# Shimly-2/DRL-on-robot-arm

Measured on AMD Instinct MI355X. Metric: env-steps/sec at N parallel envs (rl_reach_env), higher is better.
Workload: dtype f64

## Files before the change

__graft_entry__.py:

```python
import os
import subprocess
import sys

ROOT = os.path.dirname(os.path.abspath(__file__))
PKG = os.path.join(ROOT, "drl-on-robot-arm_amd")
for p in (ROOT, PKG):
    if p not in sys.path:
        sys.path.insert(0, p)


def build() -> None:
    subprocess.check_call(["make", "-C", PKG, "-j", str(min(8, os.cpu_count() or 1))], stdout=subprocess.DEVNULL)
    from oracle import oracle as _orc
    _orc.build()
    import armenv
    from armenv import _lib
    lib = _lib.load()
    assert lib.armenv_abi_version() == _lib.ABI_VERSION
    from armenv import envs


def smoke() -> None:
    import numpy as np
    import torch
    from armenv import envs
    from oracle import oracle as O

    n = 256
    env = envs.BatchedReachEnv(n, device="cuda:0", seed=1, auto_reset=False)
    assert env.kernel_name == "reach_step<f64,kuka>", env.kernel_name
    chain, cfg = O.make_chain("kuka"), O.default_config()
    st = O.ReachState(n)
    obs = env.reset().cpu().numpy()
    obs_ref = O.reach_reset(chain, cfg, st, seed=1)
    assert np.array_equal(obs[:, 3:], obs_ref[:, 3:]) and np.abs(obs - obs_ref).max() < 1e-6
# ... 19 lines not shown
```

drl-on-robot-arm_amd/armenv/envs/batched.py:

```python
import contextlib
import ctypes as C

import numpy as np
import torch

from .. import _lib as L
from ..spaces import Box
from ..urdf import Chain, builtin_chain


def _ptr(t):
    return None if t is None else C.c_void_p(t.data_ptr())


class BatchedArmEnv:

    task = L.TASK_REACH
    obs_dim = 6
    aux_dim = 0

    def __init__(self, num_envs, device="cuda:0", seed=0, auto_reset=True, precision=64, robot="kuka",
                 chain: Chain = None, env_id_offset=0, fk_path=L.FK_AUTO, **overrides):
        self._h = None
        lib = L.load()
# ... 327 lines not shown
        n, dev = self.num_envs, self.device
        ret = torch.empty(n, dtype=torch.float64, device=dev)
        ln = torch.empty(n, dtype=torch.int32, device=dev)
        su = torch.empty(n, dtype=torch.uint8, device=dev)
        with self._ordered():
            L.check(self._lib.armenv_episode_stats(self._h, _ptr(ret), _ptr(ln), _ptr(su), self._stream()))
        return ret, ln, su

    def summary(self):
        out = torch.empty(8, dtype=torch.float64, device=self.device)
        with self._ordered():
            L.check(self._lib.armenv_summary(self._h, _ptr(out), self._stream()))
        n = out[5]
        return dict(mean_distance=out[0] / n, max_distance=out[1], mean_last_return=out[2] / n, mean_last_len=out[3] / n,
                    last_success_rate=out[4] / n, raw=out)

    def counters(self):
        out = (C.c_uint64 * 16)()
        L.check(self._lib.armenv_counters(self._h, C.byref(out), self._stream()))
        return dict(episodes=out[0], successes=out[1], env_steps=out[2], nonfinite=out[3], ik_updates=out[4],
                    limit_steps=out[5], low_flange_steps=out[6], cap_steps=out[7], illcond_steps=out[8],
                    wave_trips=out[9], wave_rounds=out[10])


class BatchedReachEnv(BatchedArmEnv):
    task = L.TASK_REACH
    obs_dim = 6

    def __init__(self, num_envs, **kw):
        super().__init__(num_envs, **kw)
        lo = [0.2, -0.3, 0.0] * 2
        hi = [0.7, 0.3, 0.55] * 2
        self.observation_space = Box(low=lo, high=hi)


def diana_cam_reach_kinematics():
    import math
    big = 1.0e9
    return dict(chain=builtin_chain("diana").with_base(rpy=(0.0, 0.0, math.pi)), target_quat=[0.0, 0.0, 0.0, 1.0], dv=0.005,
                goal_lo=[0.3, -0.3, 0.0], goal_hi=[0.8, 0.3, 0.55], box_lo=[-big] * 3, box_hi=[big] * 3)


class BatchedPushEnv(BatchedArmEnv):
    task = L.TASK_PUSH
    obs_dim = 9
    aux_dim = 10
# ... 16 lines not shown
```

drl-on-robot-arm_amd/csrc/armenv_engine.h:

```cpp
#pragma once
#include <hip/hip_runtime.h>

#include <algorithm>
#include <cmath>
#include <cstdarg>
#include <cstdio>
#include <cstring>
#include <memory>
#include <new>
#include <string>
#include <type_traits>

#include "armenv_env.h"

int armenv_fail(int code, const char *fmt, ...) __attribute__((format(printf, 2, 3), visibility("hidden")));
#define fail armenv_fail

#define HIP_TRY(expr)                                                                            \
  do {                                                                                           \
    hipError_t e_ = (expr);                                                                      \
    if (e_ != hipSuccess) return fail(ARMENV_EHIP, "%s failed: %s", #expr, hipGetErrorString(e_)); \
  } while (0)

struct DeviceGuard {
// ... 62 lines not shown
                        double *trig, hipStream_t s) = 0;
  virtual int set_state(const double *q, const float *goal, const int32_t *step, const uint32_t *episode,
                        const double *ep_return, const double *aux, const double *trig, hipStream_t s) = 0;
  virtual int episode_stats(double *last_return, int32_t *last_len, uint8_t *last_success, hipStream_t s) = 0;
  virtual int episode_returns_f32(float *last_return, hipStream_t s) = 0;
  virtual int counters(uint64_t out[16], hipStream_t s) = 0;
  virtual int summary(double *out_dev, hipStream_t s) = 0;
  virtual const char *name() const = 0;
};

static inline unsigned grid_for(int64_t n, int block) { return (unsigned)((n + block - 1) / block); }

static constexpr bool fused_policy(int kind) {
  return kind == ARMENV_POLICY_ACTOR || kind == ARMENV_POLICY_ACTOR_F16X3 || kind == ARMENV_POLICY_DATD3 || kind == ARMENV_POLICY_DADDPG;
}


template <template <class, class, int> class LaneT, class C, typename T> struct Engine final : EngineBase {
  using Lane = LaneT<C, T, 0>;
  using LaneF = LaneT<C, T, 1>;
  using LaneTip = LaneT<C, T, 2>;
  bool fence_on = false;
  bool tip_on = false;
  template <bool kFused = false, class F> void with_build(bool two, F &&f) {
    auto waves = [&](auto *lane) {
      if constexpr (!kFused)
        if (two) return f(lane, std::integral_constant<int, 2>{});
      f(lane, std::integral_constant<int, 1>{});
    };
    if constexpr (kFused) waves((Lane *)nullptr);
    else if (tip_on) waves((LaneTip *)nullptr);
    else if (fence_on) waves((LaneF *)nullptr);
    else waves((Lane *)nullptr);
  }
  EnvParams<T> P{};
  void *pool = nullptr;
  unsigned long long *counter_totals = nullptr;
  double *summary_rows = nullptr;
  static constexpr int block = 256;
  int cus = 256;
  int ready_lanes = 0;
  int straggler_trips = 0;
  int waves_cfg = 0;
  int lanes_cfg = 0;
  bool half_waves() const {
    if (lanes_cfg == 64 || two_waves()) return false;
    if (lanes_cfg == 32) return true;
    return task != ARMENV_TASK_REACH && (P.n + 31) / 32 <= (int64_t)4 * cus;
  }
  static constexpr int task = Lane::kTask;
  std::string kname;

  ~Engine() override {
    if (pool) (void)hipFree(pool);
  }

// ... 70 lines not shown
      P.box_lo[k] = (T)cfg.box_lo[k]; P.box_hi[k] = (T)cfg.box_hi[k];
      K.goal_lo[k] = cfg.goal_lo[k]; K.goal_hi[k] = cfg.goal_hi[k];
    }
    double lim_min = 1e300;
    for (int j = 0; j < NJ; ++j) {
      K.q_init[j] = (T)cfg.q_init[j];
      K.lim[j] = (T)cfg.chain.limit_lo[j];
      K.lim[NJ + j] = (T)cfg.chain.limit_hi[j];
      K.lim[2 * NJ] = (T)cfg.limit_erp;
      const double a = -(double)K.lim[j], b2 = (double)K.lim[NJ + j];
      lim_min = std::fmin(lim_min, std::fmin(a, b2));
    }
    P.ik.lim = cold_dev->lim;
    P.ik.lim_min = (T)(lim_min > 0.0 ? lim_min : -1.0);
    if ((double)P.ik.lim_min > lim_min) P.ik.lim_min = std::nextafter(P.ik.lim_min, (T)0);
    for (int k = 0; k < 4; ++k) P.ik.tq[k] = (T)cfg.target_quat[k];
    P.ik.lambda = (T)cfg.ik_lambda;
    P.ik.residual = (T)cfg.ik_residual;
    P.ik.max_dtheta = (T)cfg.ik_max_dtheta;
    P.ik.max_iters = cfg.ik_max_iters;
    P.ik.exit_mode = cfg.ik_exit_mode;
    P.ik.angle_f32 = cfg.ik_angle_f32;
    P.ik.clamp_limits = cfg.clamp_joint_limits;
    waves_cfg = cfg.rollout_waves_per_simd;
    lanes_cfg = cfg.rollout_lanes_per_wave;
    ready_lanes = cfg.rollout_ready_lanes < 0 ? 0 : (cfg.rollout_ready_lanes > 64 ? 64 : cfg.rollout_ready_lanes);
    straggler_trips = cfg.rollout_straggler_trips < 0 ? 0 : cfg.rollout_straggler_trips;
    tip_on = cfg.ik_tip_offset[0] != 0.0 || cfg.ik_tip_offset[1] != 0.0 || cfg.ik_tip_offset[2] != 0.0 || cfg.fence_counters == 2;
    fence_on = cfg.fence_counters != 0 || tip_on;
    for (int k = 0; k < 3; ++k) P.ik.tip[k] = (T)cfg.ik_tip_offset[k];
    P.ik.fence_pivot = (T)cfg.fence_pivot;
    P.fence_z = (T)cfg.fence_z;
    for (int j = 0; j < NJ; ++j) {
      double R[9];
      rpy_to_mat(cfg.chain.origin_rpy[j], R);
      for (int k = 0; k < 9; ++k) P.chain.R[j][k] = (T)R[k];
      for (int k = 0; k < 3; ++k) P.chain.xyz[j][k] = (T)cfg.chain.origin_xyz[j][k];
    }
    {
      double R[9];
      rpy_to_mat(cfg.chain.base_rpy, R);
      for (int k = 0; k < 9; ++k) P.chain.base_R[k] = (T)R[k];
      for (int k = 0; k < 3; ++k) P.chain.base_p[k] = (T)cfg.chain.base_xyz[k];
    }
    HIP_TRY(hipMemcpy(cold_dev, &K, sizeof K, hipMemcpyHostToDevice));
    hipLaunchKernelGGL((trig_identity_kernel<T>), dim3(grid_for(n, block)), dim3(block), 0, 0, P);
// ... 23 lines not shown
  Launch geometry(Family f) const {
    if (f == Family::RolloutWg) return {dim3(grid_for(P.n, block)), dim3(block), P, false};
    if (two_waves()) return {dim3(grid_for(P.n, block)), dim3(block), P, true};
    const bool h = f != Family::Step && half_waves();
    const int64_t waves = h ? (P.n + 31) / 32 : (P.n + 63) / 64, per_cu = (waves + cus - 1) / cus;
    const int b = 64 * (int)std::min<int64_t>(4, std::max<int64_t>(1, per_cu));
    EnvParams<T> Q = P;
    Q.half_waves = h;
    return {dim3(grid_for(64 * waves, b)), dim3(b), Q, false};
  }
  int step(const StepIO &io, hipStream_t s) override {
    const Launch G = geometry(Family::Step);
    with_build(G.two, [&](auto *lane, auto waves) {
      using LX = std::remove_pointer_t<decltype(lane)>;
      hipLaunchKernelGGL((env_step_kernel<LX, T, decltype(waves)::value>), G.grid, G.block, 0, s, G.P, io);
    });
    HIP_TRY(hipGetLastError());
    return ARMENV_OK;
  }
  template <int POLICY>
  void launch_rollout(Family f, int32_t steps, const float *actions, const StepIO &io0, float *actions_out, hipStream_t s) {
    constexpr bool kFused = fused_policy(POLICY);
    const Launch G = geometry(f);
    with_build<kFused>(G.two, [&](auto *lane, auto waves) {
      using LX = std::remove_pointer_t<decltype(lane)>;
      constexpr int W = decltype(waves)::value;
      if constexpr (!kFused) {
        if (f == Family::RolloutAsync) {
          const int32_t ready = G.P.half_waves ? (ready_lanes + 1) / 2 : ready_lanes;
          hipLaunchKernelGGL((env_rollout_async_kernel<LX, T, POLICY, W>), G.grid, G.block, 0, s, G.P, pol, steps, actions, io0,
                             actions_out, ready, (int32_t)straggler_trips);
          return;
        }
      }
      hipLaunchKernelGGL((env_rollout_kernel<LX, T, POLICY, W>), G.grid, G.block, 0, s, G.P, pol, steps, actions, io0, actions_out);
    });
  }
  int rollout(int32_t steps, const float *actions, const StepIO &io0, float *actions_out, hipStream_t s) override {
    const Family f = ready_lanes > 0 && steps > 1 ? Family::RolloutAsync : Family::Rollout;
    if (actions) launch_rollout<ARMENV_POLICY_EXTERNAL>(f, steps, actions, io0, actions_out, s);
    else if (pol.kind == ARMENV_POLICY_ACTOR) launch_rollout<ARMENV_POLICY_ACTOR>(Family::RolloutWg, steps, actions, io0, actions_out, s);
    else if (pol.kind == ARMENV_POLICY_ACTOR_F16X3) launch_rollout<ARMENV_POLICY_ACTOR_F16X3>(Family::RolloutWg, steps, actions, io0, actions_out, s);
    else if (fused_policy(pol.kind)) launch_rollout<ARMENV_POLICY_DATD3>(Family::RolloutWg, steps, actions, io0, actions_out, s);
    else launch_rollout<ARMENV_POLICY_RANDOM>(f, steps, actions, io0, actions_out, s);
    HIP_TRY(hipGetLastError());
    return ARMENV_OK;
  }
// ... 68 lines not shown
```

drl-on-robot-arm_amd/csrc/armenv_env.h:

```cpp
#pragma once
#include "../../include/armenv.h"
#include "armenv_kin.h"
#include "armenv_actor.h"

using namespace armenv;


template <typename T> struct EnvCold {
  T q_init[NJ];
  T p_init[3];
  T trig_init[2 * NJ];
  T lim[2 * NJ + 1];
  double goal_lo[3], goal_hi[3];
  double push_rest_z, push_place_min, push_place_max, push_place_z;
  uint64_t seed, env_id0;
  int32_t push_model;
  int32_t fall_on;
  int32_t fall_land;
  T fall_c;
  T fall_keep;
  T place_z;
  T tool_radius, tool_below, erp_dt, split, fric_dv, dt;
};

// ... 55 lines not shown
    row[4] += u;
    if (l) row[5] += l;
    if (z) row[6] += z;
    if (c) row[7] += c;
    if (k) row[8] += k;
  }
}
AE_DEV uint32_t wave_max8(uint32_t v) {
  uint32_t m = 0;
  for (int b = 7; b >= 0; --b) { if (__ballot(v >= (m | (1u << b))) != 0ull) m |= 1u << b; }
  return m;
}
AE_DEV void flush_schedule(unsigned long long *counters, uint32_t wave_trips, uint32_t wave_rounds) {
  if (__ffsll((unsigned long long)__ballot(1)) - 1 == (int)(threadIdx.x & 63)) {
    unsigned long long *row = counters + kCounterCols * wave_row();
    row[9] += wave_trips;
    row[10] += wave_rounds;
  }
}
AE_DEV void flush_env_steps(unsigned long long *counters, int64_t i, unsigned long long env_steps) {
  if (i == 0) counters[2] += env_steps;
}

static __global__ __launch_bounds__(256) void counters_sum_kernel(const unsigned long long *rows, int64_t n_rows,
                                                                   unsigned long long *totals) {
  __shared__ unsigned long long part[4][kCounterCols];
  const int col = threadIdx.x & (kCounterCols - 1);
  unsigned long long acc = 0;
  for (int64_t r = threadIdx.x / kCounterCols; r < n_rows; r += 256 / kCounterCols) acc += rows[kCounterCols * r + col];
  for (int o = kCounterCols; o < 64; o <<= 1) acc += __shfl_xor(acc, o);
  if ((threadIdx.x & 63) < kCounterCols) part[threadIdx.x >> 6][col] = acc;
  __syncthreads();
  if (threadIdx.x < kCounterCols) totals[threadIdx.x] = part[0][threadIdx.x] + part[1][threadIdx.x] + part[2][threadIdx.x] + part[3][threadIdx.x];
}

struct ActionPrefetch { float x, y, z; };
AE_DEV void prefetch_issue(const float *src, ActionPrefetch &d) {
  asm volatile("global_load_dword %0, %3, off\n\tglobal_load_dword %1, %3, off offset:4\n\tglobal_load_dword %2, %3, off offset:8"
               : "=a"(d.x), "=a"(d.y), "=a"(d.z) : "v"(src) : "memory");
}
AE_DEV void prefetch_settle(ActionPrefetch &d, float (&out)[3]) {
  asm volatile("s_waitcnt vmcnt(0)\n\tv_accvgpr_read_b32 %0, %3\n\tv_accvgpr_read_b32 %1, %4\n\tv_accvgpr_read_b32 %2, %5"
               : "=v"(out[0]), "=v"(out[1]), "=v"(out[2]) : "a"(d.x), "a"(d.y), "a"(d.z) : "memory");
}

#ifndef ARMENV_TRIG_REDERIVE
// ... 265 lines not shown
        P.last_success[i] = succ ? 1 : 0;
        n_done += 1;
        if (succ) n_succ += 1;
      }
      if (done && P.auto_reset) {
        const uint32_t ep = P.episode[i];
        sample_goal(P, i, ep, g);
        P.episode[i] = ep + 1u;
        static_for<0, 3>([&](auto KI) { constexpr int k = KI; P.goal[(int64_t)k * n + i] = g[k]; });
        const EnvCold<T> &K = *P.cold;
        static_for<0, NJ>([&](auto JI) { constexpr int j = JI; q[j] = K.q_init[j]; });
        static_for<0, NJ>([&](auto JI) { constexpr int j = JI; cq[j] = K.trig_init[j]; sq[j] = K.trig_init[NJ + j]; });
        step = 0;
        ep_ret = T(0);
        store_obs6<T>(io.obs, i, K.p_init, g);
        cur_obs[0] = (float)K.p_init[0]; cur_obs[1] = (float)K.p_init[1]; cur_obs[2] = (float)K.p_init[2];
        if constexpr (CARRY) make_frame(P);
      } else if (rederive) {
        derive_trig();
        if constexpr (CARRY) make_frame(P);
      }
    }
  }
  template <bool CARRY = false, int PEEL = 0>
  AE_DEV int env_step(const EnvParams<T> &P, int64_t i, const T (&a)[3], const StepIO &io, ActionPrefetch *prefetched = nullptr,
                    float (*next_action)[3] = nullptr) {
    T tgt[3];
    step_begin<CARRY>(P, a, tgt);
    const int updates = ik_lockstep<C, T, kMode, PEEL>(P.chain, P.ik, q, tgt, S, cq, sq, minpiv);
    const bool lim_hit = ik_limits<C, T, kMode>(P.chain, P.ik, q, S, cq, sq);
    if (prefetched) prefetch_settle(*prefetched, *next_action);
    step_tail<CARRY>(P, i, io, updates, lim_hit);
    return updates;
  }

  float cur_obs[3];
  AE_DEV void refresh_obs(const EnvParams<T> &P) {
    FKState<T> F;
    fk<C, T>(P.chain, cq, sq, F);
    cur_obs[0] = (float)F.p[0]; cur_obs[1] = (float)F.p[1]; cur_obs[2] = (float)F.p[2];
  }
  AE_DEV void policy_obs(float (&s)[6]) const {
    s[0] = cur_obs[0]; s[1] = cur_obs[1]; s[2] = cur_obs[2]; s[3] = g[0]; s[4] = g[1]; s[5] = g[2];
  }
};

template <bool PICK, typename T>
AE_DEV void cube_sample(const EnvParams<T> &P, int64_t i, uint32_t episode, T (&cube)[3], T (&target)[3]) {
  const EnvCold<T> &K = *P.cold;
  double cx = 0, cy = 0, tx = 0, ty = 0, tz = K.push_place_z;
  constexpr uint32_t kBlocks = PICK ? 4u : 3u;
  for (uint32_t t = 0; t < 1000u; ++t) {
// ... 298 lines not shown
        if (succ) n_succ += 1;
      }
      if (done && P.auto_reset) {
        const uint32_t ep = P.episode[i];
        cube_sample<PICK, T>(P, i, ep, cube, target);
        P.episode[i] = ep + 1u;
        d_last = dist_ct();
        if constexpr (PICK) { grip = T(0); off[0] = off[1] = off[2] = T(0); }
        else { vel[0] = vel[1] = T(0); }
        const EnvCold<T> &K = *P.cold;
        static_for<0, NJ>([&](auto JI) { constexpr int j = JI; q[j] = K.q_init[j]; });
        static_for<0, NJ>([&](auto JI) { constexpr int j = JI; cq[j] = K.trig_init[j]; sq[j] = K.trig_init[NJ + j]; });
        step = 0;
        ep_ret = T(0);
        store_obs9<T>(io.obs, i, K.p_init, cube, target);
        cur_obs[0] = (float)K.p_init[0]; cur_obs[1] = (float)K.p_init[1]; cur_obs[2] = (float)K.p_init[2];
        if constexpr (kCarry) make_frame(P);
      } else if (rederive) {
        derive_trig();
        if constexpr (kCarry) make_frame(P);
      }
    }
  }
  template <bool CARRY = false, int PEEL = 0>
  AE_DEV int env_step(const EnvParams<T> &P, int64_t i, const T (&a)[3], const StepIO &io, ActionPrefetch *prefetched = nullptr,
                    float (*next_action)[3] = nullptr) {
    T tgt[3];
    step_begin<CARRY>(P, a, tgt);
    const int updates = ik_lockstep<C, T, kMode, PEEL>(P.chain, P.ik, q, tgt, S, cq, sq, minpiv);
    const bool lim_hit = ik_limits<C, T, kMode>(P.chain, P.ik, q, S, cq, sq);
    if (prefetched) prefetch_settle(*prefetched, *next_action);
    step_tail<CARRY>(P, i, io, updates, lim_hit);
    return updates;
  }
};
template <class C, typename T, int MODE = 0> using PushLane = CubeLane<C, T, false, MODE>;
template <class C, typename T, int MODE = 0> using PickLane = CubeLane<C, T, true, MODE>;

template <class Lane, typename T>
__global__ __launch_bounds__(256) void env_reset_kernel(EnvParams<T> P, const uint8_t *mask, const float *goal_in, float *obs) {
  const int64_t i = (int64_t)blockIdx.x * blockDim.x + threadIdx.x;
  if (i >= P.n) return;
  if (mask && !mask[i]) return;
  Lane::reset_env(P, i, goal_in, obs);
}

template <class Lane, typename T, int WAVES = 1>
__global__ __launch_bounds__(256) __attribute__((amdgpu_waves_per_eu(WAVES, WAVES))) void env_step_kernel(EnvParams<T> P, StepIO io) {
  TL_STAMP(tl0);
#ifdef ARMENV_TIMELINE
  const unsigned tl_launch = __hip_atomic_load(&g_tl_launch, __ATOMIC_RELAXED, __HIP_MEMORY_SCOPE_AGENT);
#endif
// ... 53 lines not shown
      nw = (int)(((left < (int64_t)blockDim.x ? left : (int64_t)blockDim.x) + 63) >> 6);
      if ((int)(threadIdx.x >> 6) < nw) actor_ring_init(pol.actor_h, w2_ring, nw);
    }
    __syncthreads();
  }
  const int64_t i = kActor ? (int64_t)blockIdx.x * blockDim.x + threadIdx.x : lane_env(P);
  if (i < 0) return;
  if (i >= P.n) return;
  const int64_t n = P.n;
  constexpr int kObs = Lane::kObs;
  Lane L;
  L.load(P, i);
  uint32_t episode = (POLICY != ARMENV_POLICY_EXTERNAL) ? P.episode[i] : 0u;
  if constexpr (kActor) L.refresh_obs(P);
  float an[3] = {0.f, 0.f, 0.f};
  if constexpr (kPrefetch) {
    an[0] = actions[3 * i]; an[1] = actions[3 * i + 1]; an[2] = actions[3 * i + 2];
    asm volatile("" ::"v"(an[0]), "v"(an[1]), "v"(an[2]));
  }
  ActionPrefetch an_next{0.f, 0.f, 0.f};
  [[maybe_unused]] uint32_t w_trips = 0;
  constexpr bool kCarry = !kActor;
  constexpr int kPeel = kActor ? 0 : ARMENV_ROLLOUT_PEEL;
  if constexpr (kCarry) L.make_frame(P);
  for (int32_t t = 0; t < steps; ++t) {
    T a[3];
    if constexpr (kPrefetch) {
      a[0] = (T)an[0]; a[1] = (T)an[1]; a[2] = (T)an[2];
      prefetch_issue(actions + ((int64_t)(t + 1 < steps ? t + 1 : t) * n + i) * 3, an_next);
    } else if constexpr (POLICY == ARMENV_POLICY_EXTERNAL) {
      const float *ap = actions + ((int64_t)t * n + i) * 3;
      a[0] = (T)ap[0]; a[1] = (T)ap[1]; a[2] = (T)ap[2];
    } else {
      float mu[3] = {0.f, 0.f, 0.f};
      if constexpr (POLICY == ARMENV_POLICY_ACTOR) {
        float s[kObs];
        L.policy_obs(s);
        actor_forward_wave<kObs>(pol.actor, w1_lds, s, mu);
      } else if constexpr (POLICY == ARMENV_POLICY_ACTOR_F16X3) {
        float s[kObs];
        L.policy_obs(s);
        actor_forward_wg_f16x3<kObs>(pol.actor, pol.actor_h, w1_lds, w2_ring, nw, s, mu);
      } else if constexpr (kDatd3) {
        float s[kObs], q1, q2;
        int picked;
        L.policy_obs(s);
// ... 6 lines not shown
        float v = fmaf(nz[k], pol.sigma, mu[k]);
        v = fminf(fmaxf(v, -pol.clip), pol.clip);
        a[k] = (T)v;
        an[k] = v;
      });
    }
    StepIO io;
    io.action = nullptr;
    io.obs = io0.obs + (int64_t)t * n * kObs;
    io.reward = io0.reward + (int64_t)t * n;
    io.done = io0.done + (int64_t)t * n;
    io.success = io0.success + (int64_t)t * n;
    io.terminal_obs = io0.terminal_obs ? io0.terminal_obs + (int64_t)t * n * kObs : nullptr;
    if constexpr (Lane::kFence) io.updates = io0.updates ? io0.updates + (int64_t)t * n : nullptr; else io.updates = nullptr;
    if constexpr (kTipOf(Lane::kMode)) io.diag = io0.diag ? io0.diag + (int64_t)t * n * 4 : nullptr; else io.diag = nullptr;
    if (__builtin_expect(actions_out != nullptr, 0)) {
      float *ao = actions_out + ((int64_t)t * n + i) * 3;
      if constexpr (POLICY == ARMENV_POLICY_EXTERNAL) { ao[0] = (float)a[0]; ao[1] = (float)a[1]; ao[2] = (float)a[2]; }
      else { ao[0] = an[0]; ao[1] = an[1]; ao[2] = an[2]; }
    }
    const uint32_t before = L.n_done;
    int upd;
    if constexpr (kPrefetch) {
      upd = L.template env_step<kCarry, kPeel>(P, i, a, io, &an_next, &an);
    } else {
      upd = L.template env_step<kCarry, kPeel>(P, i, a, io);
    }
    if constexpr (Lane::kFence) w_trips += wave_max8((uint32_t)upd + 1u);
    else (void)upd;
    if constexpr (POLICY != ARMENV_POLICY_EXTERNAL) {
      if (L.n_done != before && P.auto_reset) episode += 1u;
    }
  }
  L.store(P, i);
  if constexpr (kRing) actor_ring_drain();
  if constexpr (Lane::kFence) flush_schedule(P.counters, w_trips, (uint32_t)steps);
  flush_env_steps(P.counters, i, (unsigned long long)n * (unsigned long long)steps);
}

template <class Lane, typename T, int POLICY, int WAVES = 1>
__global__ __launch_bounds__(256) __attribute__((amdgpu_waves_per_eu(WAVES, WAVES)))
void env_rollout_async_kernel(EnvParams<T> P, PolicyParams pol, int32_t steps, const float *actions, StepIO io0,
                              float *actions_out, int32_t ready_lanes, int32_t straggler_trips) {
  static_assert(POLICY == ARMENV_POLICY_EXTERNAL || POLICY == ARMENV_POLICY_RANDOM, "no wave-synchronous policy phases here");
  const int64_t i = lane_env(P);
  if (i < 0) return;
  if (i >= P.n) return;
  const int64_t n = P.n;
  constexpr int kObs = Lane::kObs;
  using C = typename Lane::Chain;
  Lane L;
  L.load(P, i);
  uint32_t episode = (POLICY != ARMENV_POLICY_EXTERNAL) ? P.episode[i] : 0u;
  const T res2 = P.ik.residual * P.ik.residual;
  const bool small_steps = P.ik.max_dtheta <= T(0.7854);
  int32_t t = 0;
  bool ready = false;
  T tgt[3], diff2_prev = T(1e60);
  int updates = 0;
  float af[3] = {0.f, 0.f, 0.f};
  auto load_action = [&](int32_t tt) {
    if constexpr (POLICY == ARMENV_POLICY_EXTERNAL) {
      const float *ap = actions + ((int64_t)tt * n + i) * 3;
      af[0] = ap[0]; af[1] = ap[1]; af[2] = ap[2];
    }
  };
  auto begin_step = [&]() {
    T a[3];
    if constexpr (POLICY != ARMENV_POLICY_EXTERNAL) {
      float nz[3];
      policy_noise(P.seed, P.env_id0 + (uint64_t)i, episode - 1u, (uint32_t)L.step, nz);
      static_for<0, 3>([&](auto KI) {
        constexpr int k = KI;
        float v = nz[k] * pol.sigma;
        af[k] = fminf(fmaxf(v, -pol.clip), pol.clip);
      });
    }
    a[0] = (T)af[0]; a[1] = (T)af[1]; a[2] = (T)af[2];
    if (actions_out) {
      float *ao = actions_out + ((int64_t)t * n + i) * 3;
      ao[0] = af[0]; ao[1] = af[1]; ao[2] = af[2];
    }
    L.template step_begin<true>(P, a, tgt);
    diff2_prev = T(1e60);
    updates = 0;
    ready = false;
  };
  load_action(0);
  L.make_frame(P);
  begin_step();
  [[maybe_unused]] uint32_t w_trips = 0, w_rounds = 0;
  for (;;) {
    if constexpr (Lane::kFence) w_trips += __ballot(!ready && t < steps) != 0ull ? 1u : 0u;
    if (!ready && t < steps) ready = ik_trip<C, T, Lane::kMode>(P.chain, P.ik, L.q, tgt, L.S, L.cq, L.sq, diff2_prev, updates, res2, small_steps, L.minpiv);
    const unsigned long long rb = __ballot(ready), ib = __ballot(!ready && t < steps);
    const bool round = straggler_trips > 0 ? __ballot(!ready && t < steps && updates < straggler_trips) == 0ull : __popcll(rb) >= ready_lanes;
    if (round || ib == 0ull) {
      if constexpr (Lane::kFence) w_rounds += rb != 0ull ? 1u : 0u;
      if (ready) {
        if (t + 1 < steps) load_action(t + 1);
        const bool lim_hit = ik_limits<C, T, Lane::kMode>(P.chain, P.ik, L.q, L.S, L.cq, L.sq);
        StepIO io;
        io.action = nullptr;
        io.obs = io0.obs + (int64_t)t * n * kObs;
        io.reward = io0.reward + (int64_t)t * n;
        io.done = io0.done + (int64_t)t * n;
        io.success = io0.success + (int64_t)t * n;
        io.terminal_obs = io0.terminal_obs ? io0.terminal_obs + (int64_t)t * n * kObs : nullptr;
        if constexpr (Lane::kFence) io.updates = io0.updates ? io0.updates + (int64_t)t * n : nullptr; else io.updates = nullptr;
    if constexpr (kTipOf(Lane::kMode)) io.diag = io0.diag ? io0.diag + (int64_t)t * n * 4 : nullptr; else io.diag = nullptr;
        const uint32_t before = L.n_done;
        L.template step_tail<true>(P, i, io, updates, lim_hit);
        if constexpr (POLICY != ARMENV_POLICY_EXTERNAL) {
          if (L.n_done != before && P.auto_reset) episode += 1u;
        }
        ready = false;
        ++t;
        if (t < steps) begin_step();
      }
    }
    if (__ballot(t < steps) == 0ull) break;
  }
  L.store(P, i);
  if constexpr (Lane::kFence) flush_schedule(P.counters, w_trips, w_rounds);
  flush_env_steps(P.counters, i, (unsigned long long)n * (unsigned long long)steps);
}

template <class C, typename T>
__global__ __launch_bounds__(256) void fk_kernel(EnvParams<T> P, int64_t n, const double *q_in, double *pos, double *quat) {
  const int64_t i = (int64_t)blockIdx.x * blockDim.x + threadIdx.x;
  if (i >= n) return;
  T q[NJ];
  static_for<0, NJ>([&](auto JI) { constexpr int j = JI; q[j] = (T)q_in[7 * i + j]; });
  FKState<T> S;
  T cq[NJ], sq[NJ];
  sincos_all<T>(q, cq, sq);
  fk<C, T>(P.chain, cq, sq, S);
  static_for<0, 3>([&](auto KI) { constexpr int k = KI; pos[3 * i + k] = (double)S.p[k]; });
  if (quat) {
    T qc[4];
    quat_from_frame<T>(S.W, qc);
    static_for<0, 4>([&](auto KI) { constexpr int k = KI; quat[4 * i + k] = (double)qc[k]; });
  }
}

template <class C, typename T, int MODE = 0>
__global__ __launch_bounds__(256) void ik_kernel(EnvParams<T> P, int64_t n, const double *q_in, const double *tgt_in,
                                                 double *q_out, int32_t *iters) {
// ... 104 lines not shown
```

drl-on-robot-arm_amd/csrc/armenv_kin.h:

```cpp
#pragma once
#include "armenv_math.h"
#include "chains_builtin.h"

namespace armenv {

constexpr bool kFenceOf(int mode) { return mode >= 1; }
constexpr bool kTipOf(int mode) { return mode == 2; }

template <typename T> struct ChainDev {
  T xyz[NJ][3];
  T R[NJ][9];
  T base_p[3];
  T base_R[9];
};

struct GenericChain {
  static constexpr bool kGeneric = true;
  static constexpr const char *kName = "generic";
};

template <typename T> struct IKParams {
  T tq[4];
  T lambda;
  T residual;
  T max_dtheta;
  int32_t max_iters;
  int32_t exit_mode;
  int32_t angle_f32;
  int32_t clamp_limits;
  int32_t pad0;
// ... 218 lines not shown
template <typename T>
AE_DEV T fast_rcp(T d) {
#ifdef ARMENV_EXACT_RCP
  return T(1) / d;
#endif
  T r = hw_rcp(d);
  r = Mth<T>::fma(Mth<T>::fma(-d, r, T(1)), r, r);
  if constexpr (sizeof(T) == 8) r = Mth<T>::fma(Mth<T>::fma(-d, r, T(1)), r, r);
  return r;
}

template <typename T>
AE_DEV T fast_rsqrt(T x) {
#ifdef ARMENV_EXACT_RSQRT
  return T(1) / Mth<T>::sqrt(x);
#endif
  T r = hw_rsq(x);
  const T hx = T(0.5) * x;
  r = Mth<T>::fma(Mth<T>::fma(-hx * r, r, T(0.5)), r, r);
  if constexpr (sizeof(T) == 8) r = Mth<T>::fma(Mth<T>::fma(-hx * r, r, T(0.5)), r, r);
  return r;
}

template <typename T>
AE_DEV void quat_from_frame(const T (&W)[9], T (&q)[4]) {
  const T m00 = W[0], m10 = W[1], m20 = W[2], m01 = W[3], m11 = W[4], m21 = W[5], m02 = W[6], m12 = W[7], m22 = W[8];
  const T trace = m00 + m11 + m22;
  const bool cw = trace > T(0);
  const bool cz = !cw & (m00 < m11 ? (m11 < m22) : (m00 < m22));
  const bool cy = !cw & !cz & (m00 < m11);
  const T tw = trace + T(1), tz = m22 - m00 - m11 + T(1), ty = m11 - m22 - m00 + T(1), tx = m00 - m11 - m22 + T(1);
  const T t = cw ? tw : (cz ? tz : (cy ? ty : tx));
  const T h = T(0.5) * fast_rsqrt<T>(t);
  const T big = t * h;
  const T d21 = (m21 - m12) * h, d02 = (m02 - m20) * h, d10 = (m10 - m01) * h;
  T s10 = (m10 + m01) * h, s20 = (m20 + m02) * h, s21 = (m21 + m12) * h;
  asm("" : "+v"(s10), "+v"(s20), "+v"(s21));
  q[0] = cw ? d21 : (cz ? s20 : (cy ? s10 : big));
  q[1] = cw ? d02 : (cz ? s21 : (cy ? big : s10));
  q[2] = cw ? d10 : (cz ? big : (cy ? s21 : s20));
  q[3] = cw ? big : (cz ? d10 : (cy ? d02 : d21));
}

AE_DEV double acos_branchfree(double x) {
#ifdef ARMENV_EXACT_ACOS
  return ::acos(x);
#endif
  const double ax = ::fabs(x);
  const bool small = ax < 0.5;
  const double z = small ? x * x : ::fma(-0.5, ax, 0.5);
  double p = ::fma(3.47933107596021167570e-05, z, 7.91534994289814532176e-04);
  p = ::fma(p, z, -4.00555345006794114027e-02);
  p = ::fma(p, z, 2.01212532134862925881e-01);
  p = ::fma(p, z, -3.25565818622400915405e-01);
  p = ::fma(p, z, 1.66666666666666657415e-01);
  p = p * z;
  double q = ::fma(7.70381505559019352791e-02, z, -6.88283971605453293030e-01);
  q = ::fma(q, z, 2.02094576023350569471e+00);
  q = ::fma(q, z, -2.40339491173441421878e+00);
  q = ::fma(q, z, 1.0);
  const double R = p * fast_rcp<double>(q);
  const double sr = z * fast_rsqrt<double>(small ? 1.0 : (z > 0.0 ? z : 1.0));
  const double s = z > 0.0 ? sr : 0.0;
  const double pio2_hi = 1.57079632679489655800e+00, pio2_lo = 6.12323399573676603587e-17;
  const double inner = pio2_hi - (x - ::fma(-x, R, pio2_lo));
  const double w = ::fma(R, s, s);
  const double outer = x < 0.0 ? ::fma(-2.0, w - pio2_lo, 3.14159265358979311600e+00) : 2.0 * w;
  return small ? inner : outer;
}

template <typename T>
AE_DEV void orientation_error(const T (&tq)[4], const T (&qc)[4], int angle_f32, T (&e)[3]) {
  using M = Mth<T>;
  const T bx = -qc[0], by = -qc[1], bz = -qc[2], bw = qc[3];
  const T ax = tq[0], ay = tq[1], az = tq[2], aw = tq[3];
  const T dx = M::fma(aw, bx, M::fma(ax, bw, M::fma(ay, bz, -(az * by))));
  const T dy = M::fma(aw, by, M::fma(ay, bw, M::fma(az, bx, -(ax * bz))));
  const T dz = M::fma(aw, bz, M::fma(az, bw, M::fma(ax, by, -(ay * bx))));
  const T dw = M::fma(aw, bw, -M::fma(ax, bx, M::fma(ay, by, az * bz)));
  if constexpr (sizeof(T) == 4) {
    const T sg = dw < T(0) ? T(-1) : T(1);
    const T n = M::sqrt(M::fma(dx, dx, M::fma(dy, dy, dz * dz)));
    const T ang = T(2) * ::atan2f(n, sg * dw);
    const T k = n > T(1e-30) ? sg * ang / n : T(0);
    e[0] = k * dx; e[1] = k * dy; e[2] = k * dz;
    return;
  }
  const T wc = dw < T(-1) ? T(-1) : (dw > T(1) ? T(1) : dw);
  T angle = T(2) * (T)acos_branchfree((double)wc);
  const T s2 = M::fma(-dw, dw, T(1));
  const T v2 = M::fma(dx, dx, M::fma(dy, dy, dz * dz));
  const bool degenerate = (s2 < T(10) * M::eps) || !(v2 > T(0));
  const T rv = fast_rsqrt<T>(degenerate ? T(1) : v2);
  if (angle_f32) angle = (T)(float)angle;
  angle = angle > M::pi ? angle - T(2) * M::pi : angle;
  if (angle_f32) angle = (T)(float)angle;
  e[0] = degenerate ? angle : angle * (dx * rv);
  e[1] = degenerate ? T(0) : angle * (dy * rv);
  e[2] = degenerate ? T(0) : angle * (dz * rv);
}

template <class C, bool G = C::kGeneric> struct Axis0 { static constexpr int m = 2, sg = 1; };
template <class C> struct Axis0<C, false> { static constexpr int m = C::perm[0][2], sg = C::sgn[0][2]; };
template <class C> constexpr int k0_kind(int row) {
  if (C::kGeneric) return 0;
  const int m = Axis0<C>::m, sg = Axis0<C>::sg;
  if (row < 3) return row == m ? 1 : 0;
  return (row - 3 == m) ? (sg > 0 ? 2 : 3) : 1;
}
template <class C, bool G = C::kGeneric> struct ZKind { static constexpr int of(int, int) { return 0; } };
template <class C> struct ZKind<C, false> { static constexpr int of(int k, int r) { return FkKinds<C>().Ak[k][6 + r]; } };
template <class C> constexpr int col_kind(int k, int row) {
  if (k == 0) return k0_kind<C>(row);
  return row < 3 ? 0 : ZKind<C>::of(k, row - 3);
}
template <class C, typename T, int K, int R, int CC>
AE_DEV T jj_term(T a, T b, T acc) {
  constexpr int ka = col_kind<C>(K, R), kb = col_kind<C>(K, CC);
  if constexpr (ka == 1 || kb == 1) return acc;
  else if constexpr (ka >= 2 && kb >= 2) return acc + ((ka == kb) ? T(1) : T(-1));
  else if constexpr (ka == 2) return acc + b;
  else if constexpr (ka == 3) return acc - b;
  else if constexpr (kb == 2) return acc + a;
  else if constexpr (kb == 3) return acc - a;
  else return Mth<T>::fma(a, b, acc);
}
template <class C, typename T, int MODE = 0>
AE_DEV void dls_update(const FKState<T> &S, const T (&pe)[3], const T (&e)[6], const IKParams<T> &P, T (&dth)[NJ], T &minpiv) {
  using M = Mth<T>;
  constexpr bool FENCE = kFenceOf(MODE);
  constexpr int NL = kTipOf(MODE) ? NJ : NJ - 1;
  T Jl[NL][3];
  static_for<0, NL>([&](auto II) {
    constexpr int i = II;
    const T r0 = pe[0] - S.pj[i][0], r1 = pe[1] - S.pj[i][1], r2 = pe[2] - S.pj[i][2];
    if constexpr (i == 0 && !C::kGeneric) {
      constexpr int m = Axis0<C>::m, sg = Axis0<C>::sg;
      const T r[3] = {r0, r1, r2};
      Jl[0][m] = T(0);
      Jl[0][(m + 1) % 3] = sg > 0 ? -r[(m + 2) % 3] : r[(m + 2) % 3];
      Jl[0][(m + 2) % 3] = sg > 0 ? r[(m + 1) % 3] : -r[(m + 1) % 3];
    } else {
      constexpr int kz0 = ZKind<C>::of(i, 0), kz1 = ZKind<C>::of(i, 1), kz2 = ZKind<C>::of(i, 2);
      constexpr auto neg = [](int k) constexpr { return k < 2 ? k : (k == 2 ? 3 : 2); };
      Jl[i][0] = rot_term<kz1, neg(kz2), T>(r2, S.z[i][1], r1, -S.z[i][2]);
      Jl[i][1] = rot_term<kz2, neg(kz0), T>(r0, S.z[i][2], r2, -S.z[i][0]);
      Jl[i][2] = rot_term<kz0, neg(kz1), T>(r1, S.z[i][0], r0, -S.z[i][1]);
    }
  });
  T A[6][6];
// ... 66 lines not shown
        else if constexpr (kind == 2) { s = first ? y[r] : s + y[r]; first = false; }
        else if constexpr (kind == 3) { s = first ? -y[r] : s - y[r]; first = false; }
      });
    } else if constexpr (i < NL) {
      s = Jl[i][0] * y[0];
      s = M::fma(Jl[i][1], y[1], s);
      s = M::fma(Jl[i][2], y[2], s);
      static_for<0, 3>([&](auto RI) {
        constexpr int r = RI;
        constexpr int kz = ZKind<C>::of(i, r);
        if constexpr (kz == 0) s = M::fma(S.z[i][r], y[3 + r], s);
        else if constexpr (kz == 2) s = s + y[3 + r];
        else if constexpr (kz == 3) s = s - y[3 + r];
      });
    } else {
      s = S.z[i][0] * y[3];
      s = M::fma(S.z[i][1], y[4], s);
      s = M::fma(S.z[i][2], y[5], s);
    }
    dth[i] = s;
    mx = M::fmax(mx, M::fabs(s));
  });
  const bool over = mx > P.max_dtheta;
  const T sc = over ? P.max_dtheta * fast_rcp<T>(over ? mx : T(1)) : T(1);
  static_for<0, NJ>([&](auto II) { constexpr int i = II; dth[i] = dth[i] * sc; });
}

template <typename T, bool START_F32>
AE_DEV void ik_target(const FKState<T> &S, const T (&a)[3], T dv, const T (&box_lo)[3], const T (&box_hi)[3], T (&tgt)[3]) {
  using M = Mth<T>;
  static_for<0, 3>([&](auto KI) {
    constexpr int k = KI;
    T v = M::fma(a[k], dv, START_F32 ? (T)(float)S.p[k] : S.p[k]);
    v = v < box_lo[k] ? box_lo[k] : v;
    v = v > box_hi[k] ? box_hi[k] : v;
    tgt[k] = v;
  });
}
template <class C, typename T, int MODE = 0>
AE_DEV bool ik_stop(const IKParams<T> &P, const T (&tgt)[3], const FKState<T> &S, T diff2_prev, int it, T res2, T (&e)[6], T (&pe)[3],
                    T &diff2) {
  using M = Mth<T>;
  static_for<0, 3>([&](auto RI) {
    constexpr int r = RI;
    if constexpr (kTipOf(MODE)) pe[r] = M::fma(S.W[0 + r], P.tip[0], M::fma(S.W[3 + r], P.tip[1], M::fma(S.W[6 + r], P.tip[2], S.p[r])));
    else pe[r] = S.p[r];
  });
  e[0] = tgt[0] - pe[0];
  e[1] = tgt[1] - pe[1];
  e[2] = tgt[2] - pe[2];
  diff2 = M::fma(e[0], e[0], M::fma(e[1], e[1], e[2] * e[2]));
  int em = P.exit_mode;
  asm("" : "+v"(em));
  const T dtest = em == 0 ? diff2_prev : diff2;
  return (it >= P.max_iters) | !(dtest > res2);
}
template <class C, typename T, int MODE = 0, int SMALL = -1>
AE_DEV void ik_update(const ChainDev<T> &ch, const IKParams<T> &P, T (&q)[NJ], FKState<T> &S, T (&cq)[NJ], T (&sq)[NJ], T (&e)[6],
                      const T (&pe)[3], T diff2, T &diff2_prev, int &it, bool small_steps, T &minpiv) {
  T qc[4], eo[3], dth[NJ];
  quat_from_frame<T>(S.W, qc);
  orientation_error<T>(P.tq, qc, P.angle_f32, eo);
  e[3] = eo[0]; e[4] = eo[1]; e[5] = eo[2];
  dls_update<C, T, MODE>(S, pe, e, P, dth, minpiv);
  static_for<0, NJ>([&](auto II) { constexpr int i = II; q[i] += dth[i]; });
  if constexpr (SMALL >= 0) small_steps = SMALL != 0;
#ifdef ARMENV_EXACT_ROTATE
  small_steps = false;
#endif
  if (__builtin_expect(small_steps, 1)) {
    static_for<0, NJ>([&](auto II) { constexpr int i = II; rotate_small<T>(cq[i], sq[i], dth[i]); });
  } else {
    sincos_all<T>(q, cq, sq);
  }
  diff2_prev = diff2;
  ++it;
  fk<C, T>(ch, cq, sq, S);
}
template <class C, typename T, int MODE = 0, int SMALL = -1>
AE_DEV bool ik_trip(const ChainDev<T> &ch, const IKParams<T> &P, T (&q)[NJ], const T (&tgt)[3], FKState<T> &S, T (&cq)[NJ],
                    T (&sq)[NJ], T &diff2_prev, int &it, T res2, bool small_steps, T &minpiv) {
  T e[6], pe[3], diff2;
  if (ik_stop<C, T, MODE>(P, tgt, S, diff2_prev, it, res2, e, pe, diff2)) return true;
  ik_update<C, T, MODE, SMALL>(ch, P, q, S, cq, sq, e, pe, diff2, diff2_prev, it, small_steps, minpiv);
  return false;
}
template <class C, typename T, int MODE = 0, int PEEL = 0>
AE_DEV int ik_lockstep(const ChainDev<T> &ch, const IKParams<T> &P, T (&q)[NJ], const T (&tgt)[3], FKState<T> &S, T (&cq)[NJ],
                       T (&sq)[NJ], T &minpiv) {
  const T res2 = P.residual * P.residual;
  const bool small_steps = P.max_dtheta <= T(0.7854);
  T diff2_prev = T(1e60);
  int it = 0;
  bool stopped = false;
  static_for<0, PEEL>([&](auto) {
    if (!stopped) stopped = ik_trip<C, T, MODE>(ch, P, q, tgt, S, cq, sq, diff2_prev, it, res2, small_steps, minpiv);
  });
  if (!stopped) while (!ik_trip<C, T, MODE>(ch, P, q, tgt, S, cq, sq, diff2_prev, it, res2, small_steps, minpiv)) {}
  return it;
}

template <class C, typename T, int MODE = 0>
AE_DEV bool ik_limits(const ChainDev<T> &ch, const IKParams<T> &P, T (&q)[NJ], FKState<T> &S, T (&cq)[NJ], T (&sq)[NJ]) {
  using M = Mth<T>;
  constexpr bool FENCE = kFenceOf(MODE);
  bool hit = false;
  if (FENCE || __builtin_expect(P.clamp_limits != 0, 0)) {
    T m = M::fabs(q[0]);
    static_for<1, NJ>([&](auto II) { constexpr int i = II; m = M::fmax(m, M::fabs(q[i])); });
    if (__builtin_expect(m > P.lim_min, 0)) {
      T lo[NJ], hi[NJ];
      static_for<0, NJ>([&](auto II) { constexpr int i = II; lo[i] = P.lim[i]; hi[i] = P.lim[NJ + i]; });
      static_for<0, NJ>([&](auto II) { constexpr int i = II; hit = hit | (q[i] < lo[i]) | (q[i] > hi[i]); });
      if (P.clamp_limits && hit) {
        if (P.clamp_limits == 2) {
          const T erp = P.lim[2 * NJ];
          static_for<0, NJ>([&](auto II) {
            constexpr int i = II;
            q[i] = q[i] < lo[i] ? M::fma(erp, lo[i] - q[i], q[i]) : (q[i] > hi[i] ? M::fma(erp, hi[i] - q[i], q[i]) : q[i]);
          });
        } else {
          static_for<0, NJ>([&](auto II) { constexpr int i = II; q[i] = q[i] < lo[i] ? lo[i] : (q[i] > hi[i] ? hi[i] : q[i]); });
        }
        sincos_all<T>(q, cq, sq);
        fk<C, T>(ch, cq, sq, S);
      }
    }
  }
  return hit;
// ... 28 lines not shown
```

Before: 11.42 billion.

## Add specialized default-IK lane mode with wave-uniform fast paths in IK loop

Adds a lane mode 3 that is selected when the IK configuration matches the defaults (exit mode 0, f32 angle, small max step, no limit clamping). In this mode the exit test, small-step rotation, angle precision and limit check become compile-time constants. It also adds wave-uniform fast paths: the quaternion extraction skips the trace/z branches, acos takes only the large-argument branch, and the dtheta rescale is skipped when no lane in the wave exceeds the cap. The aim is to remove divergent selects and runtime parameter checks from the inner IK loop. The cost is extra template instantiations, a new counter column, and a changed build target.

Result: faster. 11.77 billion, median of 4 (+3.0%).

```diff
diff --git a/__graft_entry__.py b/__graft_entry__.py
--- a/__graft_entry__.py
+++ b/__graft_entry__.py
@@ -10,7 +10,7 @@
 
 
 def build() -> None:
-    subprocess.check_call(["make", "-C", PKG, "-j", str(min(8, os.cpu_count() or 1))], stdout=subprocess.DEVNULL)
+    subprocess.check_call(["make", "-C", PKG, "-j", str(min(8, os.cpu_count() or 1)), "all", "nofast"], stdout=subprocess.DEVNULL)
     from oracle import oracle as _orc
     _orc.build()
     import armenv
diff --git a/drl-on-robot-arm_amd/armenv/envs/batched.py b/drl-on-robot-arm_amd/armenv/envs/batched.py
--- a/drl-on-robot-arm_amd/armenv/envs/batched.py
+++ b/drl-on-robot-arm_amd/armenv/envs/batched.py
@@ -373,6 +373,11 @@
                     limit_steps=out[5], low_flange_steps=out[6], cap_steps=out[7], illcond_steps=out[8],
                     wave_trips=out[9], wave_rounds=out[10])
 
+    def default_ik_env_steps(self):
+        out = (C.c_uint64 * 16)()
+        L.check(self._lib.armenv_counters(self._h, C.byref(out), self._stream()))
+        return int(out[11])
+
 
 class BatchedReachEnv(BatchedArmEnv):
     task = L.TASK_REACH
diff --git a/drl-on-robot-arm_amd/csrc/armenv_engine.h b/drl-on-robot-arm_amd/csrc/armenv_engine.h
--- a/drl-on-robot-arm_amd/csrc/armenv_engine.h
+++ b/drl-on-robot-arm_amd/csrc/armenv_engine.h
@@ -108,7 +108,9 @@
   using LaneTip = LaneT<C, T, 2>;
   bool fence_on = false;
   bool tip_on = false;
-  template <bool kFused = false, class F> void with_build(bool two, F &&f) {
+  using LaneD = LaneT<C, T, 3>;
+  bool default_ik = false;
+  template <bool kFused = false, bool kRollout = false, class F> void with_build(bool two, F &&f) {
     auto waves = [&](auto *lane) {
       if constexpr (!kFused)
         if (two) return f(lane, std::integral_constant<int, 2>{});
@@ -117,7 +119,9 @@
     if constexpr (kFused) waves((Lane *)nullptr);
     else if (tip_on) waves((LaneTip *)nullptr);
     else if (fence_on) waves((LaneF *)nullptr);
-    else waves((Lane *)nullptr);
+    else if (kRollout && default_ik) {
+      if constexpr (kRollout) waves((LaneD *)nullptr);
+    } else waves((Lane *)nullptr);
   }
   EnvParams<T> P{};
   void *pool = nullptr;
@@ -234,6 +238,7 @@
     P.ik.exit_mode = cfg.ik_exit_mode;
     P.ik.angle_f32 = cfg.ik_angle_f32;
     P.ik.clamp_limits = cfg.clamp_joint_limits;
+    default_ik = P.ik.exit_mode == 0 && P.ik.angle_f32 != 0 && P.ik.max_dtheta <= T(0.7854) && P.ik.clamp_limits == 0;
     waves_cfg = cfg.rollout_waves_per_simd;
     lanes_cfg = cfg.rollout_lanes_per_wave;
     ready_lanes = cfg.rollout_ready_lanes < 0 ? 0 : (cfg.rollout_ready_lanes > 64 ? 64 : cfg.rollout_ready_lanes);
@@ -303,7 +308,7 @@
   void launch_rollout(Family f, int32_t steps, const float *actions, const StepIO &io0, float *actions_out, hipStream_t s) {
     constexpr bool kFused = fused_policy(POLICY);
     const Launch G = geometry(f);
-    with_build<kFused>(G.two, [&](auto *lane, auto waves) {
+    with_build<kFused, !kFused>(G.two, [&](auto *lane, auto waves) {
       using LX = std::remove_pointer_t<decltype(lane)>;
       constexpr int W = decltype(waves)::value;
       if constexpr (!kFused) {
diff --git a/drl-on-robot-arm_amd/csrc/armenv_env.h b/drl-on-robot-arm_amd/csrc/armenv_env.h
--- a/drl-on-robot-arm_amd/csrc/armenv_env.h
+++ b/drl-on-robot-arm_amd/csrc/armenv_env.h
@@ -101,6 +101,10 @@
   if (i == 0) counters[2] += env_steps;
 }
 
+AE_DEV void flush_default_ik_steps(unsigned long long *counters, int64_t i, unsigned long long env_steps) {
+  if (i == 0) counters[11] += env_steps;
+}
+
 static __global__ __launch_bounds__(256) void counters_sum_kernel(const unsigned long long *rows, int64_t n_rows,
                                                                    unsigned long long *totals) {
   __shared__ unsigned long long part[4][kCounterCols];
@@ -412,12 +416,12 @@
       }
     }
   }
-  template <bool CARRY = false, int PEEL = 0>
+  template <bool CARRY = false, int PEEL = 0, bool FAST = false>
   AE_DEV int env_step(const EnvParams<T> &P, int64_t i, const T (&a)[3], const StepIO &io, ActionPrefetch *prefetched = nullptr,
                     float (*next_action)[3] = nullptr) {
     T tgt[3];
     step_begin<CARRY>(P, a, tgt);
-    const int updates = ik_lockstep<C, T, kMode, PEEL>(P.chain, P.ik, q, tgt, S, cq, sq, minpiv);
+    const int updates = ik_lockstep<C, T, kMode, PEEL, FAST>(P.chain, P.ik, q, tgt, S, cq, sq, minpiv);
     const bool lim_hit = ik_limits<C, T, kMode>(P.chain, P.ik, q, S, cq, sq);
     if (prefetched) prefetch_settle(*prefetched, *next_action);
     step_tail<CARRY>(P, i, io, updates, lim_hit);
@@ -762,12 +766,12 @@
       }
     }
   }
-  template <bool CARRY = false, int PEEL = 0>
+  template <bool CARRY = false, int PEEL = 0, bool FAST = false>
   AE_DEV int env_step(const EnvParams<T> &P, int64_t i, const T (&a)[3], const StepIO &io, ActionPrefetch *prefetched = nullptr,
                     float (*next_action)[3] = nullptr) {
     T tgt[3];
     step_begin<CARRY>(P, a, tgt);
-    const int updates = ik_lockstep<C, T, kMode, PEEL>(P.chain, P.ik, q, tgt, S, cq, sq, minpiv);
+    const int updates = ik_lockstep<C, T, kMode, PEEL, FAST>(P.chain, P.ik, q, tgt, S, cq, sq, minpiv);
     const bool lim_hit = ik_limits<C, T, kMode>(P.chain, P.ik, q, S, cq, sq);
     if (prefetched) prefetch_settle(*prefetched, *next_action);
     step_tail<CARRY>(P, i, io, updates, lim_hit);
@@ -867,6 +871,7 @@
   [[maybe_unused]] uint32_t w_trips = 0;
   constexpr bool kCarry = !kActor;
   constexpr int kPeel = kActor ? 0 : ARMENV_ROLLOUT_PEEL;
+  constexpr bool kFast = !kActor && !Lane::kFence;
   if constexpr (kCarry) L.make_frame(P);
   for (int32_t t = 0; t < steps; ++t) {
     T a[3];
@@ -919,9 +924,9 @@
     const uint32_t before = L.n_done;
     int upd;
     if constexpr (kPrefetch) {
-      upd = L.template env_step<kCarry, kPeel>(P, i, a, io, &an_next, &an);
+      upd = L.template env_step<kCarry, kPeel, kFast>(P, i, a, io, &an_next, &an);
     } else {
-      upd = L.template env_step<kCarry, kPeel>(P, i, a, io);
+      upd = L.template env_step<kCarry, kPeel, kFast>(P, i, a, io);
     }
     if constexpr (Lane::kFence) w_trips += wave_max8((uint32_t)upd + 1u);
     else (void)upd;
@@ -933,6 +938,7 @@
   if constexpr (kRing) actor_ring_drain();
   if constexpr (Lane::kFence) flush_schedule(P.counters, w_trips, (uint32_t)steps);
   flush_env_steps(P.counters, i, (unsigned long long)n * (unsigned long long)steps);
+  if constexpr (Lane::kMode == 3) flush_default_ik_steps(P.counters, i, (unsigned long long)n * (unsigned long long)steps);
 }
 
 template <class Lane, typename T, int POLICY, int WAVES = 1>
@@ -951,6 +957,7 @@
   uint32_t episode = (POLICY != ARMENV_POLICY_EXTERNAL) ? P.episode[i] : 0u;
   const T res2 = P.ik.residual * P.ik.residual;
   const bool small_steps = P.ik.max_dtheta <= T(0.7854);
+  constexpr bool kFast = Lane::kMode == 3;
   int32_t t = 0;
   bool ready = false;
   T tgt[3], diff2_prev = T(1e60);
@@ -989,7 +996,7 @@
   [[maybe_unused]] uint32_t w_trips = 0, w_rounds = 0;
   for (;;) {
     if constexpr (Lane::kFence) w_trips += __ballot(!ready && t < steps) != 0ull ? 1u : 0u;
-    if (!ready && t < steps) ready = ik_trip<C, T, Lane::kMode>(P.chain, P.ik, L.q, tgt, L.S, L.cq, L.sq, diff2_prev, updates, res2, small_steps, L.minpiv);
+    if (!ready && t < steps) ready = ik_trip<C, T, Lane::kMode, -1, kFast>(P.chain, P.ik, L.q, tgt, L.S, L.cq, L.sq, diff2_prev, updates, res2, small_steps, L.minpiv);
     const unsigned long long rb = __ballot(ready), ib = __ballot(!ready && t < steps);
     const bool round = straggler_trips > 0 ? __ballot(!ready && t < steps && updates < straggler_trips) == 0ull : __popcll(rb) >= ready_lanes;
     if (round || ib == 0ull) {
@@ -1021,6 +1028,7 @@
   L.store(P, i);
   if constexpr (Lane::kFence) flush_schedule(P.counters, w_trips, w_rounds);
   flush_env_steps(P.counters, i, (unsigned long long)n * (unsigned long long)steps);
+  if constexpr (Lane::kMode == 3) flush_default_ik_steps(P.counters, i, (unsigned long long)n * (unsigned long long)steps);
 }
 
 template <class C, typename T>
diff --git a/drl-on-robot-arm_amd/csrc/armenv_kin.h b/drl-on-robot-arm_amd/csrc/armenv_kin.h
--- a/drl-on-robot-arm_amd/csrc/armenv_kin.h
+++ b/drl-on-robot-arm_amd/csrc/armenv_kin.h
@@ -4,8 +4,14 @@
 
 namespace armenv {
 
-constexpr bool kFenceOf(int mode) { return mode >= 1; }
+constexpr bool kFenceOf(int mode) { return mode == 1 || mode == 2; }
 constexpr bool kTipOf(int mode) { return mode == 2; }
+#ifdef ARMENV_NO_IK_FASTPATHS
+constexpr bool kIkFastPaths = false;
+#else
+constexpr bool kIkFastPaths = true;
+#endif
+constexpr bool kDefaultIkOf(int mode) { return kIkFastPaths && mode == 3; }
 
 template <typename T> struct ChainDev {
   T xyz[NJ][3];
@@ -270,13 +276,29 @@
   return r;
 }
 
-template <typename T>
+template <typename T, bool FAST = false>
 AE_DEV void quat_from_frame(const T (&W)[9], T (&q)[4]) {
   const T m00 = W[0], m10 = W[1], m20 = W[2], m01 = W[3], m11 = W[4], m21 = W[5], m02 = W[6], m12 = W[7], m22 = W[8];
   const T trace = m00 + m11 + m22;
   const bool cw = trace > T(0);
   const bool cz = !cw & (m00 < m11 ? (m11 < m22) : (m00 < m22));
   const bool cy = !cw & !cz & (m00 < m11);
+  if constexpr (FAST && kIkFastPaths) {
+    if (__builtin_expect(__ballot(cw | cz) == 0ull, 1)) {
+      const bool cyf = m00 < m11;
+      const T ty = m11 - m22 - m00 + T(1), tx = m00 - m11 - m22 + T(1);
+      const T t = cyf ? ty : tx;
+      const T h = T(0.5) * fast_rsqrt<T>(t);
+      const T big = t * h;
+      const T d21 = (m21 - m12) * h, d02 = (m02 - m20) * h;
+      const T s10 = (m10 + m01) * h, s20 = (m20 + m02) * h, s21 = (m21 + m12) * h;
+      q[0] = cyf ? s10 : big;
+      q[1] = cyf ? big : s10;
+      q[2] = cyf ? s21 : s20;
+      q[3] = cyf ? d02 : d21;
+      return;
+    }
+  }
   const T tw = trace + T(1), tz = m22 - m00 - m11 + T(1), ty = m11 - m22 - m00 + T(1), tx = m00 - m11 - m22 + T(1);
   const T t = cw ? tw : (cz ? tz : (cy ? ty : tx));
   const T h = T(0.5) * fast_rsqrt<T>(t);
@@ -290,11 +312,31 @@
   q[3] = cw ? big : (cz ? d10 : (cy ? d02 : d21));
 }
 
+template <bool FAST = false>
 AE_DEV double acos_branchfree(double x) {
 #ifdef ARMENV_EXACT_ACOS
   return ::acos(x);
 #endif
   const double ax = ::fabs(x);
+  if constexpr (FAST && kIkFastPaths) {
+    if (__builtin_expect(__ballot(!(x >= 0.5)) == 0ull, 1)) {
+      const double z = ::fma(-0.5, ax, 0.5);
+      double p = ::fma(3.47933107596021167570e-05, z, 7.91534994289814532176e-04);
+      p = ::fma(p, z, -4.00555345006794114027e-02);
+      p = ::fma(p, z, 2.01212532134862925881e-01);
+      p = ::fma(p, z, -3.25565818622400915405e-01);
+      p = ::fma(p, z, 1.66666666666666657415e-01);
+      p = p * z;
+      double q = ::fma(7.70381505559019352791e-02, z, -6.88283971605453293030e-01);
+      q = ::fma(q, z, 2.02094576023350569471e+00);
+      q = ::fma(q, z, -2.40339491173441421878e+00);
+      q = ::fma(q, z, 1.0);
+      const double R = p * fast_rcp<double>(q);
+      const double sr = z * fast_rsqrt<double>(z > 0.0 ? z : 1.0);
+      const double s = z > 0.0 ? sr : 0.0;
+      return 2.0 * ::fma(R, s, s);
+    }
+  }
   const bool small = ax < 0.5;
   const double z = small ? x * x : ::fma(-0.5, ax, 0.5);
   double p = ::fma(3.47933107596021167570e-05, z, 7.91534994289814532176e-04);
@@ -317,7 +359,7 @@
   return small ? inner : outer;
 }
 
-template <typename T>
+template <typename T, bool FAST = false, int ANGLE_F32 = -1>
 AE_DEV void orientation_error(const T (&tq)[4], const T (&qc)[4], int angle_f32, T (&e)[3]) {
   using M = Mth<T>;
   const T bx = -qc[0], by = -qc[1], bz = -qc[2], bw = qc[3];
@@ -334,8 +376,11 @@
     e[0] = k * dx; e[1] = k * dy; e[2] = k * dz;
     return;
   }
-  const T wc = dw < T(-1) ? T(-1) : (dw > T(1) ? T(1) : dw);
-  T angle = T(2) * (T)acos_branchfree((double)wc);
+  if constexpr (ANGLE_F32 >= 0) angle_f32 = ANGLE_F32;
+  T wc;
+  if constexpr (FAST && kIkFastPaths) wc = M::fmin(M::fmax(dw, T(-1)), T(1));
+  else wc = dw < T(-1) ? T(-1) : (dw > T(1) ? T(1) : dw);
+  T angle = T(2) * (T)acos_branchfree<FAST>((double)wc);
   const T s2 = M::fma(-dw, dw, T(1));
   const T v2 = M::fma(dx, dx, M::fma(dy, dy, dz * dz));
   const bool degenerate = (s2 < T(10) * M::eps) || !(v2 > T(0));
@@ -373,7 +418,7 @@
   else if constexpr (kb == 3) return acc - a;
   else return Mth<T>::fma(a, b, acc);
 }
-template <class C, typename T, int MODE = 0>
+template <class C, typename T, int MODE = 0, bool FAST = false>
 AE_DEV void dls_update(const FKState<T> &S, const T (&pe)[3], const T (&e)[6], const IKParams<T> &P, T (&dth)[NJ], T &minpiv) {
   using M = Mth<T>;
   constexpr bool FENCE = kFenceOf(MODE);
@@ -486,6 +531,9 @@
     mx = M::fmax(mx, M::fabs(s));
   });
   const bool over = mx > P.max_dtheta;
+  if constexpr (FAST && kIkFastPaths) {
+    if (__builtin_expect(__ballot(over) == 0ull, 1)) return;
+  }
   const T sc = over ? P.max_dtheta * fast_rcp<T>(over ? mx : T(1)) : T(1);
   static_for<0, NJ>([&](auto II) { constexpr int i = II; dth[i] = dth[i] * sc; });
 }
@@ -514,21 +562,24 @@
   e[1] = tgt[1] - pe[1];
   e[2] = tgt[2] - pe[2];
   diff2 = M::fma(e[0], e[0], M::fma(e[1], e[1], e[2] * e[2]));
+  if constexpr (kDefaultIkOf(MODE)) return (it >= P.max_iters) | !(diff2_prev > res2);
   int em = P.exit_mode;
   asm("" : "+v"(em));
   const T dtest = em == 0 ? diff2_prev : diff2;
   return (it >= P.max_iters) | !(dtest > res2);
 }
-template <class C, typename T, int MODE = 0, int SMALL = -1>
+template <class C, typename T, int MODE = 0, int SMALL = -1, bool FAST = false>
 AE_DEV void ik_update(const ChainDev<T> &ch, const IKParams<T> &P, T (&q)[NJ], FKState<T> &S, T (&cq)[NJ], T (&sq)[NJ], T (&e)[6],
                       const T (&pe)[3], T diff2, T &diff2_prev, int &it, bool small_steps, T &minpiv) {
   T qc[4], eo[3], dth[NJ];
-  quat_from_frame<T>(S.W, qc);
-  orientation_error<T>(P.tq, qc, P.angle_f32, eo);
+  constexpr bool kDef = kDefaultIkOf(MODE);
+  quat_from_frame<T, FAST>(S.W, qc);
+  orientation_error<T, FAST, kDef ? 1 : -1>(P.tq, qc, P.angle_f32, eo);
   e[3] = eo[0]; e[4] = eo[1]; e[5] = eo[2];
-  dls_update<C, T, MODE>(S, pe, e, P, dth, minpiv);
+  dls_update<C, T, MODE, FAST>(S, pe, e, P, dth, minpiv);
   static_for<0, NJ>([&](auto II) { constexpr int i = II; q[i] += dth[i]; });
-  if constexpr (SMALL >= 0) small_steps = SMALL != 0;
+  if constexpr (kDef) small_steps = true;
+  else if constexpr (SMALL >= 0) small_steps = SMALL != 0;
 #ifdef ARMENV_EXACT_ROTATE
   small_steps = false;
 #endif
@@ -541,15 +592,15 @@
   ++it;
   fk<C, T>(ch, cq, sq, S);
 }
-template <class C, typename T, int MODE = 0, int SMALL = -1>
+template <class C, typename T, int MODE = 0, int SMALL = -1, bool FAST = false>
 AE_DEV bool ik_trip(const ChainDev<T> &ch, const IKParams<T> &P, T (&q)[NJ], const T (&tgt)[3], FKState<T> &S, T (&cq)[NJ],
                     T (&sq)[NJ], T &diff2_prev, int &it, T res2, bool small_steps, T &minpiv) {
   T e[6], pe[3], diff2;
   if (ik_stop<C, T, MODE>(P, tgt, S, diff2_prev, it, res2, e, pe, diff2)) return true;
-  ik_update<C, T, MODE, SMALL>(ch, P, q, S, cq, sq, e, pe, diff2, diff2_prev, it, small_steps, minpiv);
+  ik_update<C, T, MODE, SMALL, FAST>(ch, P, q, S, cq, sq, e, pe, diff2, diff2_prev, it, small_steps, minpiv);
   return false;
 }
-template <class C, typename T, int MODE = 0, int PEEL = 0>
+template <class C, typename T, int MODE = 0, int PEEL = 0, bool FAST = false>
 AE_DEV int ik_lockstep(const ChainDev<T> &ch, const IKParams<T> &P, T (&q)[NJ], const T (&tgt)[3], FKState<T> &S, T (&cq)[NJ],
                        T (&sq)[NJ], T &minpiv) {
   const T res2 = P.residual * P.residual;
@@ -558,9 +609,9 @@
   int it = 0;
   bool stopped = false;
   static_for<0, PEEL>([&](auto) {
-    if (!stopped) stopped = ik_trip<C, T, MODE>(ch, P, q, tgt, S, cq, sq, diff2_prev, it, res2, small_steps, minpiv);
-  });
-  if (!stopped) while (!ik_trip<C, T, MODE>(ch, P, q, tgt, S, cq, sq, diff2_prev, it, res2, small_steps, minpiv)) {}
+    if (!stopped) stopped = ik_trip<C, T, MODE, -1, FAST>(ch, P, q, tgt, S, cq, sq, diff2_prev, it, res2, small_steps, minpiv);
+  });
+  if (!stopped) while (!ik_trip<C, T, MODE, -1, FAST>(ch, P, q, tgt, S, cq, sq, diff2_prev, it, res2, small_steps, minpiv)) {}
   return it;
 }
 
@@ -569,6 +620,7 @@
   using M = Mth<T>;
   constexpr bool FENCE = kFenceOf(MODE);
   bool hit = false;
+  if constexpr (kDefaultIkOf(MODE)) return hit;
   if (FENCE || __builtin_expect(P.clamp_limits != 0, 0)) {
     T m = M::fabs(q[0]);
     static_for<1, NJ>([&](auto II) { constexpr int i = II; m = M::fmax(m, M::fabs(q[i])); });
```
